# UPM-ROB-Lab/Vision-basedSensor

Hardware: AMD Instinct MI355X
Metric: frames/sec (track->3D) at 1280x1024, 169 markers (higher is better)
Workload: dtype u8+f64; 1 GPU; BASELINE config 3/4: 4096 synthetic 1280x1024 gray uint8 frames per GPU (13x13 dots, seeded jitter+noise), resident in HBM; fused track->3D table + last-seen displacement; frames_per_gpu=4096, internal_batch=1536, pass_streams=2, markers=169, channels=1, world_size=1, backend=none (single process), distinct_devices=1, tracked_observations=692224, xyz_solved=692224, ncc_ambiguous_pixels=205, ncc_exact_pixels=11244250, ncc_counter_frames=839680

## Files before the change

include/vbs.h:

```cpp
#ifndef VBS_H
#define VBS_H

#include <stdint.h>

#ifdef __cplusplus
extern "C" {
#endif

#define VBS_OK          0
#define VBS_EINVAL     -1
#define VBS_ECAPACITY  -2
#define VBS_EHIP       -3
#define VBS_ENOMEM     -4
#define VBS_EINTERNAL  -5

#define VBS_DET_COLS    6
#define VBS_TABLE_COLS 10
#define VBS_FLAG_TRACKED 1
#define VBS_FLAG_XYZ     2
#define VBS_DISP_COLS   5
#define VBS_PLANE_COLS  5
#define VBS_DEVPLANE_COLS 9

typedef struct vbs_handle vbs_handle;
// ... 22 lines not shown
int vbs_mjpeg_entropy_batch(const uint8_t* buf, const int64_t* offs, const int32_t* sizes, int n, const int32_t* info,
                            uint32_t* ent, uint32_t* tab, int64_t* frame_base, int64_t* regions, uint16_t* qt, int32_t* status,
                            int threads);
int vbs_mjpeg_reconstruct(const uint32_t* ent, const uint32_t* tab, const int64_t* frame_base, const uint16_t* qt, int n,
                          const int32_t* info, uint8_t* planes, uint8_t* out, int64_t out_frame, int64_t out_row, void* stream);
#define VBS_MJPEG_SCAN_ALIGN      16
#define VBS_MJPEG_SCAN_GUARD      16
#define VBS_MJPEG_HUFF_SET_BYTES  8928
#define VBS_MJPEG_SUBSEQ_BITS     1024
#define VBS_MJPEG_DEVICE_BITS_MAX 2147418112
#define VBS_MJPEG_SHORT           1
int vbs_mjpeg_scan_batch(const uint8_t* buf, int64_t buf_size, const int64_t* offs, const int64_t* sizes, int n, const int32_t* info,
                         uint8_t* stage, int64_t stage_cap, int64_t* scan_off, int64_t* scan_bits, int32_t* table_set, void* sets,
                         int32_t* n_sets, int64_t* regions, uint16_t* qt, int32_t* status, int threads);
int vbs_mjpeg_huffman_device(const uint8_t* stage, const int64_t* scan_off, const int64_t* scan_bits, const int32_t* table_set,
                             const void* sets, int n_sets, int n, const int32_t* info, int subseq_bits, uint32_t* ent, uint32_t* tab,
                             int64_t* frame_base, int32_t* status, void* stream);
#define VBS_JPEG_BLOCK_BITS_MAX 1660
#define VBS_JPEG_HEADER_BYTES   623
int vbs_jpeg_encode_workspace(int width, int height, int n, int64_t* workspace_bytes, int64_t* payload_bytes,
                              int64_t* frame_bound);
int vbs_jpeg_encode(const uint8_t* frames, int n, int width, int height, int64_t stride_n, int64_t stride_row, int quality,
                    void* workspace, int64_t workspace_bytes, uint8_t* payload, int64_t payload_bytes, int64_t* offsets,
                    int32_t* sizes, void* stream);
int vbs_draw_tracking(const uint8_t* frames, int n, int height, int width, int64_t stride_n, int64_t stride_row,
                      const double* det, int max_markers, const float* table, const double* ref_xy, int m_ref,
                      int32_t* lastw, uint8_t* out, void* stream);
int vbs_contour_lut(uint8_t out[256]);
int vbs_step_lut(uint32_t out[256]);
int64_t vbs_format_csv(const int64_t* frameno, const int64_t* row, const int64_t* col, const double* const* fcols, int nf,
                       int64_t n, char* buf, int64_t cap, int threads);
int vbs_gaussian_taps_q8(int ksize, double sigma, int32_t* out);
int vbs_ncc_template(int l, double sigma, double* g, double* stats);

int vbs_set_undistort(vbs_handle* h, const double* K9, const double* dist, int ndist, double* newK9, void* stream);
int vbs_undistort_frames(vbs_handle* h, const uint8_t* frames, int n, int channels, int64_t stride_n,
                         int64_t stride_row, uint8_t* out, void* stream);

int vbs_bgr2gray(vbs_handle* h, const uint8_t* frames, int n, int64_t stride_n, int64_t stride_row, uint8_t* gray,
                 void* stream);

int vbs_find_markers(vbs_handle* h, const uint8_t* frames, int n, int channels, int64_t stride_n,
                     int64_t stride_row, uint8_t* mask, uint8_t* area_mask, void* stream);

int vbs_ncc_map(vbs_handle* h, const uint8_t* frames, int n, int channels, int64_t stride_n,
                int64_t stride_row, double* ncc, void* stream);
int vbs_normxcorr2(vbs_handle* h, const uint8_t* area_mask, int n, double* ncc, uint8_t* mask,
                   void* stream);
int vbs_normxcorr2_general(int device, const double* tmpl, int th, int tw, const double* image, int h, int w, int mode,
                           double* out, void* stream);
int vbs_profile(vbs_handle* h, int enable);
int vbs_profile_read(vbs_handle* h, char* buf, int cap);
int vbs_frame_stats(vbs_handle* h, uint32_t* out, int n);
int vbs_stage_tables(vbs_handle* h, int n, uint32_t* ncomp, uint64_t* band_sums, uint32_t* area_first, int64_t* area_sums,
                     uint16_t* probe, uint32_t* slow);
int vbs_ellipse_table(vbs_handle* h, int n, double* out);
int vbs_ncc_counters(vbs_handle* h, uint64_t out[3], int reset);

int vbs_undistort_points(int device, const double* pts, int n, const vbs_camera* cam, double* out,
                         void* stream);
int vbs_calculate_3d(int device, const double* uvd, int n, const vbs_camera* cam, double* xyz,
                     int32_t* ok, void* stream);

#define VBS_PNP_SAMPLE            6
#define VBS_PNP_MAX_POINTS     1024
#define VBS_PNP_MAX_HYPOTHESES 4096
// ... 182 lines not shown
```

vision-basedsensor_amd/_lib.py:

```python
import ctypes as C
import os

_HERE = os.path.dirname(os.path.abspath(__file__))
LIB_PATH = os.path.join(_HERE, "csrc", "libvbs.so")

VBS_OK, VBS_EINVAL, VBS_ECAPACITY, VBS_EHIP, VBS_ENOMEM, VBS_EINTERNAL = 0, -1, -2, -3, -4, -5
DET_COLS, TABLE_COLS, DISP_COLS, PLANE_COLS, DEVPLANE_COLS = 6, 10, 5, 5, 9
FLAG_TRACKED, FLAG_XYZ = 1, 2
JPEG_BLOCK_BITS_MAX, JPEG_HEADER_BYTES = 1660, 623
MJPEG_SCAN_ALIGN, MJPEG_SCAN_GUARD, MJPEG_HUFF_SET_BYTES, MJPEG_SUBSEQ_BITS, MJPEG_SHORT = 16, 16, 8928, 1024, 1
SERIES_CHUNK, SERIES_REC_COLS, STATS_COLS, WINDOW_COLS = 32, 5, 5, 4
FIR_MAX_TAPS, FIR_TILE, AXIS_COLS, TOTAL_COLS = 255, 64, 4, 5
STEP_MAX_WINDOW, STEP_MAX_STEPS = 64, 64
POSE_COLS, POSEFIELD_COLS, POSE_GROUP = 8, 6, 8
FIELD_FRAMES, FIELD_MAX_SLOTS, FIELD_MAX_POINTS, PATCH_COLS, PATCH_GROUP = 4, 1024, 65536, 8, 8
PROJ_SLOTS, PROJ_CHUNK, PROJ_ROWS, PROJ_WG_SLOTS, PROJ_MAX_ROWS, PROJ_MAX_FRAMES, PROJ_MAX_SLOTS = 4, 64, 64, 16, 8192, 1048576, 1024
FIT_GROUP, PEAK_COLS = 4, 7
ENV_TILE, ENV_MAX_HALF = 64, 127
MOM_CHUNK, MOM_WG_SLOTS, MOM_MAX_SLOTS = 32, 16, 1024
MODES_MAX, MODES_MAX_DIM, MODES_SWEEPS, MODES_MAX_ITERS, SCORE_GROUP = 16, 3072, 10, 4096, 8
STRAIN_COLS, LSTRAIN_COLS, MOTION_GROUP, LSTRAIN_GROUP, STRAIN_MAX_NBR = 16, 8, 8, 8, 12
ROBUST_MAX_HALF, ROBUST_TILE = 31, 64
DIAM_COLS, DIAM_STATS_COLS, DIAM_MAX_EXTENT = 24, 5, 512
PNP_SAMPLE, PNP_MAX_POINTS, PNP_MAX_HYPOTHESES, PNP_FEW_POINTS, PNP_NO_HYPOTHESIS = 6, 1024, 4096, 1, 2
CHESS_MAX_CANDIDATES, CHESS_MAX_PATTERN, CHESS_MAX_WIN = 256, 256, 15
CALIB_MAX_VIEWS, CALIB_FEW_VIEWS, CALIB_DEGENERATE = 64, 1, 2
IDS_MAX_MARKERS, IDS_MAX_LAYERS = 1024, 16
OPT_GRAY_COEFFS, OPT_FORCE_SEQ_MATCH, OPT_NCC_MARGIN, OPT_STAGE_IMPL, OPT_BLUR_IMPL, OPT_PASS_STREAMS, OPT_LATENCY_FRAMES = 1, 2, 4, 5, 6, 7, 8

SYMBOLS = ("vbs_create", "vbs_destroy", "vbs_last_error", "vbs_version", "vbs_contour_lut",
           "vbs_gaussian_taps_q8", "vbs_ncc_template", "vbs_set_undistort", "vbs_undistort_frames", "vbs_find_markers", "vbs_ncc_map", "vbs_normxcorr2",
           "vbs_profile", "vbs_profile_read", "vbs_frame_stats", "vbs_undistort_points", "vbs_calculate_3d", "vbs_marker_center",
           "vbs_track", "vbs_solve3d", "vbs_track_to_3d", "vbs_displacement", "vbs_displacement_range", "vbs_displacement_f64",
           "vbs_plane_fit", "vbs_assign_ids", "vbs_set_option", "vbs_bgr2gray", "vbs_ncc_counters", "vbs_normxcorr2_general",
           "vbs_stage_tables", "vbs_ellipse_table", "vbs_deviation_plane", "vbs_format_csv", "vbs_mjpeg_probe", "vbs_mjpeg_entropy_batch",
           "vbs_mjpeg_reconstruct", "vbs_jpeg_encode_workspace", "vbs_jpeg_encode", "vbs_draw_tracking",
           "vbs_series_chunks", "vbs_series_stats", "vbs_series_stats_f64", "vbs_series_partial", "vbs_series_merge",
           "vbs_window_means", "vbs_displacement_from_frame", "vbs_mjpeg_scan_batch", "vbs_mjpeg_huffman_device",
           "vbs_step_lut", "vbs_threshold_bits", "vbs_measure_markers", "vbs_pnp_ransac",
           "vbs_chess_workspace", "vbs_chess_corners", "vbs_corner_subpix", "vbs_calibrate_camera",
           "vbs_axis_displacement", "vbs_fir_series_f64",
           "vbs_step_response_f64", "vbs_find_steps_f64", "vbs_dwell_stats_f64", "vbs_pose_series",
           "vbs_field_map_f64", "vbs_patch_stats_f64", "vbs_project_series_f64", "vbs_harmonic_fit_f64", "vbs_window_moments_f64", "vbs_window_fit_f64",
           "vbs_motion_series_f64", "vbs_local_strain_f64", "vbs_hampel_series_f64",
           "vbs_cross_moments_f64", "vbs_covariance_f64", "vbs_leading_modes_f64", "vbs_mode_scores_f64")


class Camera(C.Structure):
    _fields_ = [("K", C.c_float * 9), ("dist", C.c_float * 5), ("R", C.c_float * 9),
                ("T", C.c_float * 3), ("marker_diameter_mm", C.c_float)]


class VbsError(RuntimeError):
    pass


def status_text(status: int, max_markers: int = 0) -> str:
    if status == VBS_ECAPACITY:
        return ("the frame exceeds the device workspace (more than 30720 runs in a mask, more than "
                f"{max_markers or 'max_markers'} band components, more than about 512 contours, or a contour thousands of rows "
                "long whose vertex moments would leave 64 bits)")
    if status == VBS_EINTERNAL:
        return ("a kernel's internal hand-shake timed out: the frame's result is not to be trusted (bounded wait expired; "
                "see VBS_EINTERNAL in include/vbs.h)")
    return "unexpected device status"


_lib = None


def lib():
    global _lib
    if _lib is not None:
        return _lib
    if not os.path.exists(LIB_PATH):
        raise VbsError(f"{LIB_PATH} is missing: build it with `python -c 'import __graft_entry__ as g; "
                       f"g.build()'` (hipcc, gfx950). There is no CPU fallback.")
    try:
        import torch
    except ImportError:
        pass
    L = C.CDLL(LIB_PATH)
    vp, i32, i64, f64 = C.c_void_p, C.c_int, C.c_int64, C.c_double
    cam_p = C.POINTER(Camera)
    sig = {
        "vbs_create": (i32, [i32, i32, i32, i32, i32, C.POINTER(vp)]),
        "vbs_destroy": (i32, [vp]),
        "vbs_last_error": (C.c_char_p, [vp]),
        "vbs_version": (i32, []),
        "vbs_contour_lut": (i32, [vp]),
        "vbs_gaussian_taps_q8": (i32, [i32, f64, vp]),
        "vbs_ncc_template": (i32, [i32, f64, vp, vp]),
        "vbs_set_undistort": (i32, [vp, vp, vp, i32, vp, vp]),
        "vbs_undistort_frames": (i32, [vp, vp, i32, i32, i64, i64, vp, vp]),
        "vbs_find_markers": (i32, [vp, vp, i32, i32, i64, i64, vp, vp, vp]),
        "vbs_ncc_map": (i32, [vp, vp, i32, i32, i64, i64, vp, vp]),
        "vbs_normxcorr2": (i32, [vp, vp, i32, vp, vp, vp]),
        "vbs_profile": (i32, [vp, i32]),
        "vbs_profile_read": (i32, [vp, vp, i32]),
        "vbs_frame_stats": (i32, [vp, vp, i32]),
        "vbs_undistort_points": (i32, [i32, vp, i32, cam_p, vp, vp]),
        "vbs_calculate_3d": (i32, [i32, vp, i32, cam_p, vp, vp, vp]),
        "vbs_marker_center": (i32, [vp, vp, vp, i32, vp, vp, vp]),
        "vbs_track": (i32, [vp, vp, vp, i32, vp, i32, f64, vp, vp]),
        "vbs_solve3d": (i32, [vp, vp, i32, i32, cam_p, f64, vp]),
        "vbs_track_to_3d": (i32, [vp, vp, i32, i32, i64, i64, vp, i32, f64, cam_p, f64, vp, vp, vp, vp]),
        "vbs_displacement": (i32, [vp, vp, i32, i32, i32, f64, f64, vp, vp]),
        "vbs_displacement_range": (i32, [vp, vp, i32, i32, i32, f64, f64, i32, i32, vp, vp]),
        "vbs_displacement_f64": (i32, [i32, vp, i32, i32, i32, f64, f64, vp, vp]),
        "vbs_plane_fit": (i32, [vp, vp, i32, i32, vp, vp]),
        "vbs_assign_ids": (i32, [vp, vp, vp, i32, i32, vp, vp, i32, vp, vp]),
        "vbs_set_option": (i32, [vp, i32, i32]),
        "vbs_bgr2gray": (i32, [vp, vp, i32, i64, i64, vp, vp]),
        "vbs_ncc_counters": (i32, [vp, vp, i32]),
        "vbs_normxcorr2_general": (i32, [i32, vp, i32, i32, vp, i32, i32, i32, vp, vp]),
        "vbs_stage_tables": (i32, [vp, i32, vp, vp, vp, vp, vp, vp]),
        "vbs_ellipse_table": (i32, [vp, i32, vp]),
        "vbs_deviation_plane": (i32, [vp, vp, vp, vp, vp, vp, i32, i32, f64, vp, vp, vp]),
        "vbs_format_csv": (i64, [vp, vp, vp, vp, i32, i64, vp, i64, i32]),
        "vbs_mjpeg_probe": (i32, [vp, i64, vp]),
        "vbs_mjpeg_entropy_batch": (i32, [vp, vp, vp, i32, vp, vp, vp, vp, vp, vp, vp, i32]),
        "vbs_mjpeg_reconstruct": (i32, [vp, vp, vp, vp, i32, vp, vp, vp, i64, i64, vp]),
        "vbs_mjpeg_scan_batch": (i32, [vp, i64, vp, vp, i32, vp, vp, i64, vp, vp, vp, vp, vp, vp, vp, vp, i32]),
        "vbs_mjpeg_huffman_device": (i32, [vp, vp, vp, vp, vp, i32, i32, vp, i32, vp, vp, vp, vp, vp]),
        "vbs_jpeg_encode_workspace": (i32, [i32, i32, i32, vp, vp, vp]),
# ... 57 lines not shown
```

vision-basedsensor_amd/csrc/api.hip:

```cpp
#include <algorithm>
#include <cmath>
#include <cstring>
#include <new>

#include "common.h"

static std::vector<int> gaussian_taps_q8(int ksize, double sigma) {
    std::vector<double> v(ksize);
    const double scale2x = -0.125 / (sigma * sigma);
    for (int i = 0; i < ksize; ++i) {
        double xi = (double)(1 - ksize + 2 * i);
        v[i] = std::exp(xi * xi * scale2x);
    }
    const int n2 = (ksize - 1) / 2;
    double s = 0;
    for (int i = 0; i < n2; ++i) s += v[i];
    s = 2.0 * s + 1.0;
    const double mul = 1.0 / s;
    std::vector<int> out(ksize, 0);
    double err = 0;
    int tot = 0;
    for (int i = 0; i < ksize / 2; ++i) {
        double adj = v[i] * mul * 256.0 + err;
        int v0 = (int)std::nearbyint(adj);
// ... 42 lines not shown
    h->allocs.push_back(q);
    *p = (T*)q;
    return VBS_OK;
}

extern "C" int vbs_version(void) { return 100; }

extern "C" int vbs_contour_lut(uint8_t out[256]) {
    if (!out) return VBS_EINVAL;
    make_contour_lut(out);
    return VBS_OK;
}

extern "C" int vbs_step_lut(uint32_t out[256]) {
    if (!out) return VBS_EINVAL;
    make_step_lut(out);
    return VBS_OK;
}

extern "C" int vbs_gaussian_taps_q8(int ksize, double sigma, int32_t* out) {
    if (!out || ksize < 1 || !(ksize & 1) || !(sigma > 0)) return VBS_EINVAL;
    std::vector<int> k = gaussian_taps_q8(ksize, sigma);
    for (int i = 0; i < ksize; ++i) out[i] = k[i];
    return VBS_OK;
}

extern "C" int vbs_ncc_template(int l, double sigma, double* g, double* stats) {
    if (!g || !stats || l < 2 || l > VBS_NCC_MAXL || !(sigma > 0)) return VBS_EINVAL;
    NccConst nc;
    ncc_consts(l, sigma, &nc);
    for (int i = 0; i < l; ++i) g[i] = nc.g[i];
    stats[0] = nc.tbar; stats[1] = nc.T2; stats[2] = nc.l2; stats[3] = nc.thr2;
    return VBS_OK;
}

extern "C" int vbs_destroy(vbs_handle* h) {
    if (!h) return VBS_EINVAL;
    (void)hipSetDevice(h->device);
    if (h->stream2) (void)hipStreamDestroy(h->stream2);
    if (h->ev_fork) (void)hipEventDestroy(h->ev_fork);
    if (h->ev_join) (void)hipEventDestroy(h->ev_join);
    for (void* p : h->allocs) (void)hipFree(p);
    if (h->series_ws) (void)hipFree(h->series_ws);
    delete h;
    return VBS_OK;
}

extern "C" const char* vbs_last_error(const vbs_handle* h) { return h ? h->err.c_str() : "null handle"; }

static int alloc_workspace(vbs_handle* h, Workspace& w) {
    const size_t B = (size_t)h->maxb, M = (size_t)h->maxm, HW = (size_t)h->H * h->WW;
    int rc;
#define ALLOC(field, count) if ((rc = dev_alloc(h, &w.field, (count))) != VBS_OK) return rc
    ALLOC(area_bits, B * HW); ALLOC(mask_bits, B * HW); ALLOC(band_bits, B * HW);
    ALLOC(open_bits, B * HW);
    ALLOC(wbase, B * 2 * HW);
    if (2 * HW < (size_t)16 * SG_REC) ALLOC(stage_mrec, B * 16 * SG_REC);
    ALLOC(node_pos, B * 2 * VBS_RUN_CAP); ALLOC(node_comp, B * 2 * VBS_RUN_CAP);
    ALLOC(ncomp, B * 2);
    ALLOC(band_first, B * M); ALLOC(band_sums, B * M * 4);
    ALLOC(area_first, B * M); ALLOC(area_sums, B * M * VBS_AREA_SUMS);
    ALLOC(ell, B * M * 8); ALLOC(det64, B * M * 6);
    ALLOC(cnt, B);
    ALLOC(probe, B * M * 4); ALLOC(ncc_tot, 4);
    ALLOC(lat_hdr, (size_t)VBS_LAT_MAXN * VBS_LAT_HDR + 4 + B + B * 8 + 8);
#undef ALLOC
// ... 60 lines not shown
    std::vector<double> rx(width), ry(height);
    for (int x = 0; x < width; ++x) {
        double s = 0;
        for (int j = 0; j < bp.ncc_l; ++j) { int xx = x + bp.ncc_lo + j; if (xx >= 0 && xx < width) s += h->ncc.g[j]; }
        rx[x] = s;
    }
    for (int y = 0; y < height; ++y) {
        double s = 0;
        for (int j = 0; j < bp.ncc_l; ++j) { int yy = y + bp.ncc_lo + j; if (yy >= 0 && yy < height) s += h->ncc.g[j]; }
        ry[y] = s;
    }
    u8 lut[256];
    make_contour_lut(lut);
    HIPCHK(h, hipMemcpy(h->ncc_rx, rx.data(), width * sizeof(double), hipMemcpyHostToDevice));
    HIPCHK(h, hipMemcpy(h->ncc_ry, ry.data(), height * sizeof(double), hipMemcpyHostToDevice));
    HIPCHK(h, hipMemcpy(h->lut, lut, 256, hipMemcpyHostToDevice));
    u32 steps[256];
    make_step_lut(steps);
    HIPCHK(h, hipMemcpy(h->step_lut, steps, sizeof(steps), hipMemcpyHostToDevice));
    HIPCHK(h, hipMemcpy(h->blur_frags, frags.data(), frags.size() * sizeof(u32), hipMemcpyHostToDevice));
    if (h->blur16_h) {
        HIPCHK(h, hipMemcpy(h->blur16_h, frags16h.data(), frags16h.size() * sizeof(u32), hipMemcpyHostToDevice));
        HIPCHK(h, hipMemcpy(h->blur16_v, frags16v.data(), frags16v.size() * sizeof(u32), hipMemcpyHostToDevice));
    }
    HIPCHK(h, hipMemcpy(h->ncc_frags, nfrags.data(), nfrags.size() * sizeof(u32), hipMemcpyHostToDevice));
    {
        std::vector<float2> rowf(height);
        for (int y = 0; y < height; ++y) {
            const int ny = std::min(y + bp.ncc_hi, height - 1) - std::max(y + bp.ncc_lo, 0) + 1;
            rowf[y] = make_float2((float)ny, (float)ry[y]);
        }
        HIPCHK(h, hipMemcpy(h->ncc_rowf, rowf.data(), height * sizeof(float2), hipMemcpyHostToDevice));
    }
    HIPCHK(h, hipMemcpy(h->ncc_tab, h->ncc.g, VBS_NCC_MAXL * sizeof(double), hipMemcpyHostToDevice));
    HIPCHK(h, hipMemcpy(h->ncc_tab + VBS_NCC_MAXL, h->ncc.cg, (VBS_NCC_MAXL + 1) * sizeof(double), hipMemcpyHostToDevice));
    {
        std::vector<int32_t> wt(4096);
        bilinear_weights_i16(wt.data());
        HIPCHK(h, hipMemcpy(h->uwtab, wt.data(), 4096 * sizeof(int32_t), hipMemcpyHostToDevice));
    }
    if ((rc = alloc_workspace(h, h->ws[0])) != VBS_OK) return rc;
    HIPCHK(h, hipDeviceSynchronize());
    return VBS_OK;
}

static int check_launch(vbs_handle* h) {
    hipError_t e = hipGetLastError();
    if (e != hipSuccess) { h->err = std::string("kernel launch: ") + hipGetErrorString(e); return VBS_EHIP; }
    return VBS_OK;
}

static bool capturing(hipStream_t s) {
    hipStreamCaptureStatus st = hipStreamCaptureStatusNone;
    return hipStreamIsCapturing(s, &st) == hipSuccess && st != hipStreamCaptureStatusNone;
}

static int need_gray(vbs_handle* h, Workspace& w, hipStream_t s) {
    const size_t bytes = (size_t)h->maxb * h->H * h->P;
    if (!w.gray) {
        if (capturing(s)) {
            h->err = "the gray plane of 3-channel / undistorted input is allocated at first use: run one such call (or "
                     "vbs_set_undistort) outside stream capture first";
            return VBS_EINVAL;
        }
        int rc = dev_alloc(h, &w.gray, bytes);
        if (rc != VBS_OK) return rc;
// ... 981 lines not shown
```

vision-basedsensor_amd/csrc/common.h:

```cpp
#pragma once
#include <hip/hip_runtime.h>
#include <stdint.h>
#include <string>
#include <vector>

#include "../../include/vbs.h"

typedef unsigned long long u64;
typedef long long i64;
typedef uint32_t u32;
typedef uint8_t u8;

#define VBS_NCC_MAXL 80
#define VBS_RUN_CAP 30720
#define VBS_AREA_SUMS 16
#define VBS_LAT_MAXN 32
#define VBS_LAT_HDR 128
#define VBS_WINDOWS_PER_LAUNCH 16

struct BranchParams {
    int taps_a, taps_b;
    int thresh, hi;
    int ncc_l;
    int ncc_lo, ncc_hi;
// ... 36 lines not shown
    u32* node_comp;
    u32* ncomp;
    u32* band_first;
    u64* band_sums;
    u32* area_first;
    i64* area_sums;
    double* ell;
    double* det64;
    int32_t* cnt;
    unsigned short* probe;
    u64* ncc_tot;
    u32* lat_hdr;
    u32* slow_total;
    u32* slow_flag;
    u32* fstat;
    unsigned char* lat_scratch = nullptr;
    int lat_slots = 0;
};

struct vbs_handle {
    bool prof = false;
    std::vector<ProfRec> recs;
    int device, H, W, P, WW, maxm, maxb;
    BranchParams bp;
    NccConst ncc;
    std::string err;
    uint4* blur_frags;
    uint4* blur16_h = nullptr;
    uint4* blur16_v = nullptr;
    double* ncc_rx;
    double* ncc_ry;
    uint4* ncc_frags;
    float2* ncc_rowf;
    double* ncc_tab;
    u8* lut;
    u32* step_lut = nullptr;
    short* umap1;
    unsigned short* umap2;
    int* uwtab;
    bool undist = false;
    double newK[9];
    int blur_impl = 0;
    int pass_streams = 2;
    int stage_impl = 0;
    int gray_bits = 15;
    bool force_seq_match = false;
    int ncc_margin_ppm = 0;
    int lat_frames = 24;
    size_t stage_lds_set[2] = {0, 0}, ccl_lds_set[2] = {0, 0}, lat_lds_set = 0;
    Workspace ws[2];
    int nws = 1;
    Workspace* last_ws = ws;
    hipStream_t stream2 = nullptr;
    hipEvent_t ev_fork = nullptr, ev_join = nullptr;
    std::vector<void*> allocs;
    double* series_ws = nullptr;
    size_t series_cap = 0;
};

static inline int series_chunks(int n, int frame_begin) {
    return (int)(((int64_t)frame_begin + n - 1) / VBS_SERIES_CHUNK - frame_begin / VBS_SERIES_CHUNK + 1);
}

#define HIPCHK(h, call)                                                                   \
    do {                                                                                  \
        hipError_t e_ = (call);                                                           \
// ... 138 lines not shown
```

vision-basedsensor_amd/csrc/k_ncc_mfma.hip:

```cpp
#include <algorithm>
#include <cstddef>
#include <cstring>
#include <type_traits>

#include "ncc_common.h"

typedef _Float16 h8 __attribute__((ext_vector_type(8)));
typedef _Float16 h4 __attribute__((ext_vector_type(4)));
typedef float f4 __attribute__((ext_vector_type(4)));
typedef float f2 __attribute__((ext_vector_type(2)));
typedef int i4 __attribute__((ext_vector_type(4)));
typedef __attribute__((address_space(1))) u8 gl_u8;
typedef __attribute__((address_space(1))) unsigned short gl_u16;

template <int L> struct NccLit;
template <> struct NccLit<80> { static constexpr float kc = 163.84f, ks2 = 547.2815085234848f, K1 = 3502601.654550303f; };
template <> struct NccLit<33> { static constexpr float kc = 962.8797061524332f, ks2 = 6956.564407359948f, K1 = 7575698.639614983f; };

struct NccKArgs {
    const u64* bits; const double* rx; const double* ry; const uint4* wfrag; const double* tab; const float2* rowf;
    u64* mbits; u8* mask_u8; u32* fstat; u64* tot;
    int H, W, WW, tiles_per_seg, dbg_arg; float rel_arg;
    NccConst nc;
};
typedef __attribute__((address_space(4))) const NccKArgs NccKArgsC;
__device__ __forceinline__ NccKArgsC* ncc_kargs() {
    NccKArgsC* p = (NccKArgsC*)__builtin_amdgcn_kernarg_segment_ptr();
    asm volatile("" : "+s"(p));
    return p;
}

template <int L, int LO, bool U8OUT>
__global__ __launch_bounds__(256, 4) void k_ncc_mfma(const u64* __restrict__ bits, const double* __restrict__ rx,
                                                     const double* __restrict__ ry, const uint4* __restrict__ wfrag,
                                                     const double* __restrict__ tab, const float2* __restrict__ rowf,
                                                     u64* __restrict__ mbits, u8* __restrict__ mask_u8,
                                                     u32* __restrict__ fstat, u64* __restrict__ tot, int H, int W, int WW,
                                                     int tiles_per_seg,
                                                     int dbg_arg, float rel_arg, NccConst nc) {
#ifdef VBS_DEBUG_KNOBS
    const int dbg = dbg_arg;
#else
    constexpr int dbg = 0;
#endif
    constexpr int HI = L - 1 + LO;
    constexpr int NT = (16 + L - 1 + 15) / 16;
    constexpr int NKS = (16 * NT + 31) / 32;
    constexpr int NK8 = (16 * NT + 63) / 64;
    constexpr int RING = 16 * NT;
    constexpr int RSTR = RING + 8;
    constexpr int CSTR = RING + 16;
    constexpr int ECAP = 2 * NT + 2;
    __shared__ struct __align__(16) {
        uint4 lut[256];
        _Float16 ring[4][2][16 * RSTR];
        u8 ringc[4][16 * CSTR];
        u32 elist[4][ECAP][10];
    } sm;
    const int tid = threadIdx.x, lane = tid & 63;
    const int wave = __builtin_amdgcn_readfirstlane(tid >> 6);
    const int g = lane >> 4, q = lane & 15;
    const int n = blockIdx.z;
    const int tilesY = (H + 15) / 16;
    const int tile0 = blockIdx.y * tiles_per_seg;
    const int ntiles = min(tiles_per_seg, tilesY - tile0);
    if (ntiles <= 0) return;
    const int Y0 = tile0 * 16, nsteps = ntiles + NT - 1;
    const int xw = blockIdx.x * 64 + 16 * wave;
    const u64* fbits = bits + (int64_t)n * H * WW;
    {
        u32 w[4];
#pragma unroll
        for (int d = 0; d < 4; ++d) w[d] = (((u32)tid >> (2 * d)) & 1u ? 0x3C00u : 0u) | (((u32)tid >> (2 * d + 1)) & 1u ? 0x3C000000u : 0u);
        sm.lut[tid] = make_uint4(w[0], w[1], w[2], w[3]);
    }
    for (int i = lane; i < 2 * 16 * RSTR / 8; i += 64) reinterpret_cast<uint4*>(&sm.ring[wave][0][0])[i] = make_uint4(0, 0, 0, 0);
    for (int i = lane; i < 16 * CSTR / 16; i += 64) reinterpret_cast<uint4*>(&sm.ringc[wave][0])[i] = make_uint4(0, 0, 0, 0);
    h8 whi[NKS], wlo[NKS], one[NKS];
#pragma unroll
    for (int s = 0; s < NKS; ++s) {
        uint4 a = wfrag[(0 * NKS + s) * 64 + lane], b = wfrag[(1 * NKS + s) * 64 + lane], c = wfrag[(2 * NKS + s) * 64 + lane];
        whi[s] = __builtin_bit_cast(h8, a);
        wlo[s] = __builtin_bit_cast(h8, b);
        one[s] = __builtin_bit_cast(h8, c);
    }
    i4 one8[NK8];
#pragma unroll
    for (int s = 0; s < NK8; ++s) {
        const uint4 a = wfrag[(3 * NKS + s) * 64 + lane];
        one8[s] = i4{(int)a.x, (int)a.y, (int)a.z, (int)a.w};
    }
    __builtin_amdgcn_s_waitcnt(0x0F70);
    __syncthreads();

    const double mu = (double)(255ull * (u64)fstat[n * 8 + 0]) / (double)((int64_t)H * W);
    const double full_t = ry[min(max(-LO, 0), H - 1)] * rx[min(max(-LO, 0), W - 1)];
    auto uni = [](float v) { float o; asm("s_nop 4\n\tv_readfirstlane_b32 %0, %1\n\ts_nop 4" : "=s"(o) : "v"(v)); return o; };
    const float kc = uni((float)(nc.tbar * (NCC_WSCALE * NCC_WSCALE)));
    const float th0 = (float)ncc_theta(0.0, nc.l2, full_t, mu, nc);
    bool lit_ok;
    {
        const double ksd = sqrt(nc.thr2 * nc.T2) / (double)L * (NCC_WSCALE * NCC_WSCALE);
        const double k0d = mu * (full_t - nc.l2 * nc.tbar) / 255.0 * (NCC_WSCALE * NCC_WSCALE);
        lit_ok = fabs(nc.tbar * (NCC_WSCALE * NCC_WSCALE) - (double)NccLit<L>::kc) <= 2e-7 * (double)NccLit<L>::kc &&
                 fabs(ksd * ksd - (double)NccLit<L>::ks2) <= 2e-7 * (double)NccLit<L>::ks2 && fabs(k0d) < 1e-4;
    }
    const bool th0pos = __builtin_amdgcn_readfirstlane((th0 > 0.0f && lit_ok) ? 1 : 0) != 0;
    const bool xin = (xw + LO >= 0) && (xw + 15 + HI <= W - 1);
#ifdef VBS_DEBUG_KNOBS
    const int plain_lo = dbg == 10 ? -0x40000000 : (th0pos && xin && dbg != 11) ? -LO : 0x7FFFFFFF, plain_hi = dbg == 10 ? 0x40000000 : H - 1 - 15 - HI;
#else
    const int plain_lo = (th0pos && xin) ? -LO : 0x7FFFFFFF, plain_hi = H - 1 - 15 - HI;
#endif
    const int valid_hi = (xw + 15 < W) ? H - 16 : -1;
    const float muf = uni((float)mu), tbarf = uni((float)nc.tbar), ktf = uni((float)(nc.tbar * 255.0)), il2f = uni((float)nc.inv_l2);
    const float krf = uni((float)(nc.thr2 * nc.T2));
    const float mukf = uni((float)(mu / 255.0 * (NCC_WSCALE * NCC_WSCALE)));
    const int xq = min(xw + q, W - 1);
    const float nxf = (float)(min(xq + HI, W - 1) - max(xq + LO, 0) + 1), rxf = (float)rx[xq];
    const float nnc = (float)L * nxf, stc = (float)ry[min(max(-LO, 0), H - 1)] * rxf, dd0c = stc - nnc * tbarf;
    _Float16* const ringw = &sm.ring[wave][0][q * RSTR];
    _Float16* const wr = ringw + 4 * g;
    const _Float16* const rd = ringw + 8 * g;
// ... 126 lines not shown
                    double rhs = d_nc_thr2 * var * d_nc_T2;
                    double num = 255.0 * Ge + rest;
                    const int flags = __builtin_amdgcn_readfirstlane((var > 0.0 ? 1 : 0) | ((var > 0.0 && num > 0.0 && num * num > rhs) ? 2 : 0) |
                                                                     ((var > 1e-6 && num > 0.0 && fabs(num * num - rhs) <= 1e-9 * rhs) ? 4 : 0));
                    if ((flags & 2) && lane == 0) {
                        atomicOr(&mb32[(u32)__mul24(y, 2 * d_WW) + (u32)(xe >> 5)], 1u << (xe & 31));
                        if (U8OUT) d_mask_u8[((int64_t)n * d_H + y) * d_W + xe] = 1;
                    }
                    if (flags & 1) { nexact++; if (flags & 4) amb++; }
                }
            }
        }
        ecnt = 0;
    };
    h8 a_op[NKS];
    auto fetch_ops = [&](int tt) {
        u32 by[NKS];
        const u32 rw[5] = {nraw.x, nraw.y, nraw.z, nraw.w, 0u};
#pragma unroll
        for (int s = 0; s < NKS; ++s) by[s] = __builtin_amdgcn_perm(rw[s + 1], rw[s], psel);
#pragma unroll
        for (int s = 0; s < NKS; ++s) asm volatile("" : "+v"(by[s]) :: "memory");
        load_rows(tt + 1);
        flush_pending();
        const int ytile = Y0 + LO + 16 * tt;
        if (ytile < 0 || ytile + 15 >= H) {
            const bool rowin = (ytile + q >= 0) && (ytile + q < H);
#pragma unroll
            for (int s = 0; s < NKS; ++s) by[s] = rowin ? by[s] : 0u;
        }
#pragma unroll
        for (int s = 0; s < NKS; ++s) a_op[s] = __builtin_bit_cast(h8, sm.lut[by[s]]);
    };
    load_rows(0);
    fetch_ops(0);
    for (int t0 = 0; t0 < nsteps; t0 += NT) {
#pragma unroll
        for (int u = 0; u < NT; ++u) {
            const int t = t0 + u;
            if (t >= nsteps) break;
            constexpr int dummy_nt = NT;
            const int B = (u + 1) % dummy_nt;
            constexpr int NKE = (RING - 16) / 32;
            constexpr int NK8E = (RING - 16) / 64;
            f4 G = {0, 0, 0, 0};
            i4 C = {0, 0, 0, 0};
            auto vert_f16 = [&](int s) {
                const int r0 = (16 * B + 32 * s) % RING;
                const _Float16* p = (r0 + 32 <= RING ? rd : rdw) + r0;
                const h8 bh = *reinterpret_cast<const h8*>(p);
                const h8 bl = *reinterpret_cast<const h8*>(p + LOFS);
                G = __builtin_amdgcn_mfma_f32_16x16x32_f16(whi[s], bh, G, 0, 0, 0);
                G = __builtin_amdgcn_mfma_f32_16x16x32_f16(whi[s], bl, G, 0, 0, 0);
                G = __builtin_amdgcn_mfma_f32_16x16x32_f16(wlo[s], bh, G, 0, 0, 0);
            };
            auto vert_i8 = [&](int s) {
                const int gi = min(4 * s + g, NT - 1);
                const int slot = B + gi - (gi >= NT - B ? NT : 0);
                const i4 bc = *reinterpret_cast<const i4*>(cbase + 16 * slot);
                C = __builtin_amdgcn_mfma_i32_16x16x64_i8(one8[s], bc, C, 0, 0, 0);
            };
            const bool vert = !(t < NT - 1 || dbg == 3);
            f4 ah = {0, 0, 0, 0}, ac = {0, 0, 0, 0};
            if (vert) {
#pragma unroll
                for (int s = 0; s < NKS; ++s) {
                    ah = __builtin_amdgcn_mfma_f32_16x16x32_f16(a_op[s], whi[s], ah, 0, 0, 0);
                    if (s < NKE) vert_f16(s);
// ... 182 lines not shown
    for (int s = 0; s < nk8; ++s)
        for (int lane = 0; lane < 64; ++lane)
            for (int j = 0; j < 16; ++j) {
                const int idx = 64 * s + 16 * (lane >> 4) + j - (lane & 15);
                if (idx >= 0 && idx < l) out[((size_t)(3 * nks + s) * 64 + lane) * 4 + (j >> 2)] |= 1u << (8 * (j & 3));
            }
    auto bits16 = [](double v) { _Float16 hv = (_Float16)v; unsigned short b; memcpy(&b, &hv, 2); return (u32)b; };
    for (int kind = 0; kind < 3; ++kind)
        for (int s = 0; s < nks; ++s)
            for (int lane = 0; lane < 64; ++lane) {
                const int g = lane >> 4, col = lane & 15;
                for (int j = 0; j < 8; ++j) {
                    const int idx = 32 * s + 8 * g + j - col;
                    u32 v = 0;
                    if (idx >= 0 && idx < l) {
                        const double w = nc.g[idx] * NCC_WSCALE;
                        const _Float16 hi = (_Float16)w;
                        v = kind == 0 ? bits16((double)hi) : kind == 1 ? bits16(w - (double)hi) : bits16(1.0);
                    }
                    out[((size_t)(kind * nks + s) * 64 + lane) * 4 + (j >> 1)] |= v << (16 * (j & 1));
                }
            }
    return out;
}

void launch_ncc_mfma(vbs_handle* h, Workspace& w, int nb, u8* mask_u8, hipStream_t s) {
    const int tilesY = (h->H + 15) / 16;
    const int want = h->WW * nb <= 512 ? 1024 : 2048;
    int nseg = std::min(tilesY, std::max(1, want == 1024 ? want / (h->WW * nb) : (want + h->WW * nb - 1) / (h->WW * nb)));
    if (VBS_KNOB("VBS_NCC_NSEG")) nseg = VBS_KNOB("VBS_NCC_NSEG");
    const int tps = (tilesY + nseg - 1) / nseg;
    nseg = (tilesY + tps - 1) / tps;
    dim3 grid(h->WW, nseg, nb);
#define NCC_GO(L_, LO_, U8)                                                                                      \
    VBS_LAUNCH(h, s, "k_ncc_mfma", (k_ncc_mfma<L_, LO_, U8>), grid, dim3(256), 0, s, w.area_bits, h->ncc_rx,     \
               h->ncc_ry, h->ncc_frags, h->ncc_tab, h->ncc_rowf, w.mask_bits, mask_u8, w.fstat, w.ncc_tot,       \
               h->H, h->W, h->WW, tps,                                                                           \
               VBS_KNOB("VBS_NCC_DBG"), std::max(NCC_REL, 1e-6f * (float)h->ncc_margin_ppm), h->ncc)
    if (!h->bp.small) { if (mask_u8) NCC_GO(80, -40, true); else NCC_GO(80, -40, false); }
    else { if (mask_u8) NCC_GO(33, -16, true); else NCC_GO(33, -16, false); }
#undef NCC_GO
}
```

vision-basedsensor_amd/csrc/ncc_common.h:

```cpp
#pragma once
#include "common.h"

__device__ __forceinline__ u64 load_bits(const u64* __restrict__ row, int WW, int start) {
    int wi = start >> 6, sh = start & 63;
    u64 a = (wi >= 0 && wi < WW) ? row[wi] : 0ull;
    u64 b = (wi + 1 >= 0 && wi + 1 < WW) ? row[wi + 1] : 0ull;
    return sh ? ((a >> sh) | (b << (64 - sh))) : a;
}

template <int L, int LO>
__device__ __forceinline__ double ncc_row_exact(const u64* __restrict__ row, int WW, int x, const double* cg,
                                                u32* cnt) {
    u64 w0 = load_bits(row, WW, x + LO), w1 = 0;
    if (L > 64) w1 = load_bits(row, WW, x + LO + 64) & ((1ull << (L > 64 ? L - 64 : 1)) - 1ull);
    else w0 &= (1ull << (L < 64 ? L : 0)) - 1ull;
    *cnt += __popcll(w0) + __popcll(w1);
    double h = 0.0;
#pragma unroll
    for (int half = 0; half < 2; ++half) {
        u64 w = half ? w1 : w0;
        while (w) {
            int b0 = __ffsll((long long)w) - 1;
            u64 t = ~(w >> b0);
            int len = t ? __ffsll((long long)t) - 1 : 64 - b0;
            w &= (len >= 64) ? 0ull : ~(((1ull << len) - 1ull) << b0);
            h += cg[half * 64 + b0 + len] - cg[half * 64 + b0];
        }
    }
    return h;
}

template <int L, int LO>
__device__ __attribute__((noinline)) double ncc_exact_G(const u64* fbits, int H, int WW, int y, int x, const double* cg,
                                                        const double* gsh) {
    u32 dummy = 0;
    double Ge = 0.0;
    for (int i = 0; i < L; ++i) {
        int yy = y + LO + i;
        double hrow = (yy >= 0 && yy < H) ? ncc_row_exact<L, LO>(fbits + (int64_t)yy * WW, WW, x, cg, &dummy) : 0.0;
        Ge = __builtin_fma(gsh[i], hrow, Ge);
    }
    return Ge;
}

#define NCC_WSCALE 1024.0
#define NCC_REL 2e-5f
#define NCC_NEVER 3e38
#define NCC_ABS 1e-3f

__device__ __forceinline__ double ncc_theta(double c, double nn, double sum_t, double mu, const NccConst& nc) {
    double sum_I = 255.0 * c;
    double rest = -nc.tbar * sum_I - mu * (sum_t - nn * nc.tbar);
    double s1 = sum_I - nn * mu;
    double s2 = 255.0 * sum_I - 2.0 * mu * sum_I + nn * mu * mu;
    double var = s2 - s1 * s1 * nc.inv_l2;
    double rhs = nc.thr2 * var * nc.T2;
    if (!(var > 0.0)) return NCC_NEVER;
    if (c == 0.0) return (rest > 0.0 && rest * rest > rhs) ? -NCC_NEVER : NCC_NEVER;
    return (sqrt(rhs) - rest) * (NCC_WSCALE * NCC_WSCALE / 255.0);
}
```

Before: 292,400 frames/s.

## Trim NCC MFMA tile range to rows with occupied area bits

Adds a pre-scan in the NCC MFMA kernel that ballots over the wave's column window to find the first and last input rows holding set area bits. It shrinks the tile range to the rows that window can influence, and zeroes mask output outside that range directly. A host-side guard decides from the template constants whether empty windows can be safely treated as non-matches, and the trim is enabled only when the guard passes. The aim is to skip MFMA correlation work over blank regions of the frame, at the cost of an extra pass of bit loads and some setup code per block.

Measured after the change: 315,200 frames/s, median of 6. 1.08x the previous value.

```diff
diff --git a/include/vbs.h b/include/vbs.h
--- a/include/vbs.h
+++ b/include/vbs.h
@@ -78,6 +78,7 @@
                        int64_t n, char* buf, int64_t cap, int threads);
 int vbs_gaussian_taps_q8(int ksize, double sigma, int32_t* out);
 int vbs_ncc_template(int l, double sigma, double* g, double* stats);
+int vbs_ncc_trim_guard(int l, double sigma, int height, int width, double tbar_shift, double* min_d0);
 
 int vbs_set_undistort(vbs_handle* h, const double* K9, const double* dist, int ndist, double* newK9, void* stream);
 int vbs_undistort_frames(vbs_handle* h, const uint8_t* frames, int n, int channels, int64_t stride_n,
diff --git a/vision-basedsensor_amd/_lib.py b/vision-basedsensor_amd/_lib.py
--- a/vision-basedsensor_amd/_lib.py
+++ b/vision-basedsensor_amd/_lib.py
@@ -29,7 +29,7 @@
 OPT_GRAY_COEFFS, OPT_FORCE_SEQ_MATCH, OPT_NCC_MARGIN, OPT_STAGE_IMPL, OPT_BLUR_IMPL, OPT_PASS_STREAMS, OPT_LATENCY_FRAMES = 1, 2, 4, 5, 6, 7, 8
 
 SYMBOLS = ("vbs_create", "vbs_destroy", "vbs_last_error", "vbs_version", "vbs_contour_lut",
-           "vbs_gaussian_taps_q8", "vbs_ncc_template", "vbs_set_undistort", "vbs_undistort_frames", "vbs_find_markers", "vbs_ncc_map", "vbs_normxcorr2",
+           "vbs_gaussian_taps_q8", "vbs_ncc_template", "vbs_ncc_trim_guard", "vbs_set_undistort", "vbs_undistort_frames", "vbs_find_markers", "vbs_ncc_map", "vbs_normxcorr2",
            "vbs_profile", "vbs_profile_read", "vbs_frame_stats", "vbs_undistort_points", "vbs_calculate_3d", "vbs_marker_center",
            "vbs_track", "vbs_solve3d", "vbs_track_to_3d", "vbs_displacement", "vbs_displacement_range", "vbs_displacement_f64",
            "vbs_plane_fit", "vbs_assign_ids", "vbs_set_option", "vbs_bgr2gray", "vbs_ncc_counters", "vbs_normxcorr2_general",
@@ -91,6 +91,7 @@
         "vbs_contour_lut": (i32, [vp]),
         "vbs_gaussian_taps_q8": (i32, [i32, f64, vp]),
         "vbs_ncc_template": (i32, [i32, f64, vp, vp]),
+        "vbs_ncc_trim_guard": (i32, [i32, f64, i32, i32, f64, vp]),
         "vbs_set_undistort": (i32, [vp, vp, vp, i32, vp, vp]),
         "vbs_undistort_frames": (i32, [vp, vp, i32, i32, i64, i64, vp, vp]),
         "vbs_find_markers": (i32, [vp, vp, i32, i32, i64, i64, vp, vp, vp]),
diff --git a/vision-basedsensor_amd/csrc/api.hip b/vision-basedsensor_amd/csrc/api.hip
--- a/vision-basedsensor_amd/csrc/api.hip
+++ b/vision-basedsensor_amd/csrc/api.hip
@@ -98,6 +98,36 @@
     for (int i = 0; i < l; ++i) g[i] = nc.g[i];
     stats[0] = nc.tbar; stats[1] = nc.T2; stats[2] = nc.l2; stats[3] = nc.thr2;
     return VBS_OK;
+}
+
+static double ncc_trim_guard(const NccConst& nc, int l, int height, int width, double tbar_shift) {
+    const int lo = -((l - 1) - (l - 1) / 2);
+    auto cuts = [&](int size) {
+        std::vector<std::pair<int, double>> out;
+        for (int p = 0; p < size; ++p) {
+            if (p == l && size - l > l) p = size - l;
+            double s = 0;
+            int cnt = 0;
+            for (int j = 0; j < l; ++j) { const int pp = p + lo + j; if (pp >= 0 && pp < size) { s += nc.g[j]; ++cnt; } }
+            out.emplace_back(cnt, s);
+        }
+        return out;
+    };
+    const auto rows = cuts(height), cols = cuts(width);
+    double mn = 1e300;
+    for (const auto& r : rows)
+        for (const auto& c : cols) mn = std::min(mn, r.second * c.second - (double)(r.first * c.first) * (nc.tbar + tbar_shift));
+    return mn;
+}
+static constexpr double NCC_TRIM_SLACK = -5e-5;
+
+extern "C" int vbs_ncc_trim_guard(int l, double sigma, int height, int width, double tbar_shift, double* min_d0) {
+    if (l < 2 || l > VBS_NCC_MAXL || !(sigma > 0) || height < 1 || width < 1) return VBS_EINVAL;
+    NccConst nc;
+    ncc_consts(l, sigma, &nc);
+    const double mn = ncc_trim_guard(nc, l, height, width, tbar_shift);
+    if (min_d0) *min_d0 = mn;
+    return mn > NCC_TRIM_SLACK ? 1 : 0;
 }
 
 extern "C" int vbs_destroy(vbs_handle* h) {
@@ -224,6 +254,7 @@
         }
         HIPCHK(h, hipMemcpy(h->ncc_rowf, rowf.data(), height * sizeof(float2), hipMemcpyHostToDevice));
     }
+    h->ncc_trim_ok = ncc_trim_guard(h->ncc, bp.ncc_l, height, width, 0.0) > NCC_TRIM_SLACK;
     HIPCHK(h, hipMemcpy(h->ncc_tab, h->ncc.g, VBS_NCC_MAXL * sizeof(double), hipMemcpyHostToDevice));
     HIPCHK(h, hipMemcpy(h->ncc_tab + VBS_NCC_MAXL, h->ncc.cg, (VBS_NCC_MAXL + 1) * sizeof(double), hipMemcpyHostToDevice));
     {
diff --git a/vision-basedsensor_amd/csrc/common.h b/vision-basedsensor_amd/csrc/common.h
--- a/vision-basedsensor_amd/csrc/common.h
+++ b/vision-basedsensor_amd/csrc/common.h
@@ -92,6 +92,7 @@
     double* ncc_ry;
     uint4* ncc_frags;
     float2* ncc_rowf;
+    bool ncc_trim_ok = false;
     double* ncc_tab;
     u8* lut;
     u32* step_lut = nullptr;
diff --git a/vision-basedsensor_amd/csrc/k_ncc_mfma.hip b/vision-basedsensor_amd/csrc/k_ncc_mfma.hip
--- a/vision-basedsensor_amd/csrc/k_ncc_mfma.hip
+++ b/vision-basedsensor_amd/csrc/k_ncc_mfma.hip
@@ -39,7 +39,7 @@
                                                      int tiles_per_seg,
                                                      int dbg_arg, float rel_arg, NccConst nc) {
 #ifdef VBS_DEBUG_KNOBS
-    const int dbg = dbg_arg;
+    const int dbg = dbg_arg & (NCC_TRIM_BIT - 1);
 #else
     constexpr int dbg = 0;
 #endif
@@ -63,9 +63,9 @@
     const int n = blockIdx.z;
     const int tilesY = (H + 15) / 16;
     const int tile0 = blockIdx.y * tiles_per_seg;
-    const int ntiles = min(tiles_per_seg, tilesY - tile0);
+    int ntiles = min(tiles_per_seg, tilesY - tile0);
     if (ntiles <= 0) return;
-    const int Y0 = tile0 * 16, nsteps = ntiles + NT - 1;
+    int Y0 = tile0 * 16;
     const int xw = blockIdx.x * 64 + 16 * wave;
     const u64* fbits = bits + (int64_t)n * H * WW;
     {
@@ -74,21 +74,77 @@
         for (int d = 0; d < 4; ++d) w[d] = (((u32)tid >> (2 * d)) & 1u ? 0x3C00u : 0u) | (((u32)tid >> (2 * d + 1)) & 1u ? 0x3C000000u : 0u);
         sm.lut[tid] = make_uint4(w[0], w[1], w[2], w[3]);
     }
-    for (int i = lane; i < 2 * 16 * RSTR / 8; i += 64) reinterpret_cast<uint4*>(&sm.ring[wave][0][0])[i] = make_uint4(0, 0, 0, 0);
-    for (int i = lane; i < 16 * CSTR / 16; i += 64) reinterpret_cast<uint4*>(&sm.ringc[wave][0])[i] = make_uint4(0, 0, 0, 0);
+    if (dbg_arg & NCC_TRIM_BIT) {
+        const int seg_y0 = Y0, seg_y1 = min(Y0 + 16 * ntiles, H);
+        const int r0 = max(Y0 + LO, 0), r1 = min(Y0 + 16 * ntiles - 1 + HI, H - 1);
+        const int pws = xw + LO, pb0 = pws >> 3;
+        const bool pwide = (pb0 >= 0) && ((pb0 & ~3) + 16 <= 8 * WW);
+        constexpr int NB = 16 + L - 1;
+        int first = 0x7FFFFFFF, last = -1;
+        for (int base = r0; base <= r1; base += 256) {
+            u64 w0[4], w1[4];
+#pragma unroll
+            for (int k = 0; k < 4; ++k) {
+                const int row = min(base + 64 * k + lane, r1);
+                if (pwide) {
+                    const uint4 rr = *reinterpret_cast<const uint4*>(reinterpret_cast<const u8*>(fbits) + (pb0 & ~3) + (int64_t)row * (8 * WW));
+                    const u64 lo64 = (u64)rr.x | ((u64)rr.y << 32), hi64 = (u64)rr.z | ((u64)rr.w << 32);
+                    const int sh = 8 * (pb0 & 3);
+                    w0[k] = sh ? (lo64 >> sh) | (hi64 << (64 - sh)) : lo64;
+                    w1[k] = hi64 >> sh;
+                } else {
+                    const u64* prow = fbits + (int64_t)row * WW;
+                    w0[k] = load_bits(prow, WW, pws);
+                    w1[k] = NB > 64 ? load_bits(prow, WW, pws + 64) : 0ull;
+                }
+            }
+#pragma unroll
+            for (int k = 0; k < 4; ++k) {
+                const u64 v0 = NB >= 64 ? w0[k] : w0[k] & ((1ull << (NB & 63)) - 1ull);
+                const u64 v1 = NB > 64 ? w1[k] & ((1ull << ((NB - 64) & 63)) - 1ull) : 0ull;
+                const u64 occ = __ballot((v0 | v1) != 0ull);
+                if (occ) {
+                    first = min(first, min(base + 64 * k + (int)__builtin_ctzll(occ), r1));
+                    last = max(last, min(base + 64 * k + 63 - (int)__builtin_clzll(occ), r1));
+                }
+            }
+        }
+        int ta = tile0;
+        if (last >= 0) {
+            const int tb = min(Y0 + 16 * ntiles - 1, last - LO) >> 4;
+            ta = max(Y0, first - HI) >> 4;
+            ntiles = tb - ta + 1;
+        } else {
+            ntiles = 0;
+        }
+        Y0 = 16 * __builtin_amdgcn_readfirstlane(ta);
+        ntiles = __builtin_amdgcn_readfirstlane(ntiles);
+        u8* zb = reinterpret_cast<u8*>(reinterpret_cast<unsigned short*>(mbits) + ((int64_t)n * H * WW + blockIdx.x) * 4 + wave);
+        for (int y = seg_y0 + lane; y < seg_y1; y += 64)
+            if (y < Y0 || y >= Y0 + 16 * ntiles) *reinterpret_cast<unsigned short*>(zb + (int64_t)y * (8 * WW)) = 0;
+        if (U8OUT) {
+            for (int y = seg_y0 + g; y < seg_y1; y += 4)
+                if ((y < Y0 || y >= Y0 + 16 * ntiles) && xw + q < W) mask_u8[((int64_t)n * H + y) * W + xw + q] = 0;
+        }
+    }
+    const int nsteps = ntiles > 0 ? ntiles + NT - 1 : 0;
     h8 whi[NKS], wlo[NKS], one[NKS];
-#pragma unroll
-    for (int s = 0; s < NKS; ++s) {
-        uint4 a = wfrag[(0 * NKS + s) * 64 + lane], b = wfrag[(1 * NKS + s) * 64 + lane], c = wfrag[(2 * NKS + s) * 64 + lane];
-        whi[s] = __builtin_bit_cast(h8, a);
-        wlo[s] = __builtin_bit_cast(h8, b);
-        one[s] = __builtin_bit_cast(h8, c);
-    }
     i4 one8[NK8];
-#pragma unroll
-    for (int s = 0; s < NK8; ++s) {
-        const uint4 a = wfrag[(3 * NKS + s) * 64 + lane];
-        one8[s] = i4{(int)a.x, (int)a.y, (int)a.z, (int)a.w};
+    if (nsteps) {
+        for (int i = lane; i < 2 * 16 * RSTR / 8; i += 64) reinterpret_cast<uint4*>(&sm.ring[wave][0][0])[i] = make_uint4(0, 0, 0, 0);
+        for (int i = lane; i < 16 * CSTR / 16; i += 64) reinterpret_cast<uint4*>(&sm.ringc[wave][0])[i] = make_uint4(0, 0, 0, 0);
+#pragma unroll
+        for (int s = 0; s < NKS; ++s) {
+            uint4 a = wfrag[(0 * NKS + s) * 64 + lane], b = wfrag[(1 * NKS + s) * 64 + lane], c = wfrag[(2 * NKS + s) * 64 + lane];
+            whi[s] = __builtin_bit_cast(h8, a);
+            wlo[s] = __builtin_bit_cast(h8, b);
+            one[s] = __builtin_bit_cast(h8, c);
+        }
+#pragma unroll
+        for (int s = 0; s < NK8; ++s) {
+            const uint4 a = wfrag[(3 * NKS + s) * 64 + lane];
+            one8[s] = i4{(int)a.x, (int)a.y, (int)a.z, (int)a.w};
+        }
     }
     __builtin_amdgcn_s_waitcnt(0x0F70);
     __syncthreads();
@@ -281,8 +337,10 @@
 #pragma unroll
         for (int s = 0; s < NKS; ++s) a_op[s] = __builtin_bit_cast(h8, sm.lut[by[s]]);
     };
-    load_rows(0);
-    fetch_ops(0);
+    if (nsteps) {
+        load_rows(0);
+        fetch_ops(0);
+    }
     for (int t0 = 0; t0 < nsteps; t0 += NT) {
 #pragma unroll
         for (int u = 0; u < NT; ++u) {
@@ -531,11 +589,12 @@
     const int tps = (tilesY + nseg - 1) / nseg;
     nseg = (tilesY + tps - 1) / tps;
     dim3 grid(h->WW, nseg, nb);
+    const int trim = (h->ncc_trim_ok && !VBS_KNOB("VBS_NCC_DBG") && !VBS_KNOB("VBS_NCC_TRIM_OFF")) ? NCC_TRIM_BIT : 0;
 #define NCC_GO(L_, LO_, U8)                                                                                      \
     VBS_LAUNCH(h, s, "k_ncc_mfma", (k_ncc_mfma<L_, LO_, U8>), grid, dim3(256), 0, s, w.area_bits, h->ncc_rx,     \
                h->ncc_ry, h->ncc_frags, h->ncc_tab, h->ncc_rowf, w.mask_bits, mask_u8, w.fstat, w.ncc_tot,       \
                h->H, h->W, h->WW, tps,                                                                           \
-               VBS_KNOB("VBS_NCC_DBG"), std::max(NCC_REL, 1e-6f * (float)h->ncc_margin_ppm), h->ncc)
+               VBS_KNOB("VBS_NCC_DBG") | trim, std::max(NCC_REL, 1e-6f * (float)h->ncc_margin_ppm), h->ncc)
     if (!h->bp.small) { if (mask_u8) NCC_GO(80, -40, true); else NCC_GO(80, -40, false); }
     else { if (mask_u8) NCC_GO(33, -16, true); else NCC_GO(33, -16, false); }
 #undef NCC_GO
diff --git a/vision-basedsensor_amd/csrc/ncc_common.h b/vision-basedsensor_amd/csrc/ncc_common.h
--- a/vision-basedsensor_amd/csrc/ncc_common.h
+++ b/vision-basedsensor_amd/csrc/ncc_common.h
@@ -46,6 +46,7 @@
 #define NCC_WSCALE 1024.0
 #define NCC_REL 2e-5f
 #define NCC_NEVER 3e38
+#define NCC_TRIM_BIT 0x100
 #define NCC_ABS 1e-3f
 
 __device__ __forceinline__ double ncc_theta(double c, double nn, double sum_t, double mu, const NccConst& nc) {
```
